# filrg/attackFL

Hardware: AMD Instinct MI355X
Metric: FL rounds/sec (whole node) + test-acc, TransformerModel/ICU, 8 clients (higher is better)
Workload: dtype bf16; 1 GPU; model=TransformerModel, global_batch=1024, seq_len=1, parallelism=fl8-clients-over-1-ranks, clients=8, local_epochs=5, rows_per_client=12000-15000, mode=fedavg, trainer=fused

## Files before the change

### attackfl_amd/fl/trainers.py

```python
from __future__ import annotations

from dataclasses import dataclass
from typing import List, Optional, Sequence, Tuple

import time

import torch

from ..data import DeviceTable
from ..models import ParamLayout, build_model
from ..utils.log import print_with_color


@dataclass
class Plan:

    order: torch.Tensor
    nd: torch.Tensor
    epochs: int
    nd_dev: Optional[torch.Tensor] = None

    def client(self, c: int) -> torch.Tensor:
        return self.order[c, :, : int(self.nd[c])]

# ... 288 lines not shown

        def fin():
            while not done.query():
                time.sleep(0)
            okh = buf[:, 0].to(torch.int32)
            if bool((okh < 0).any()):
                raise RuntimeError(f"{what}: a cross-workgroup hand-off timed out (workgroups not co-resident?)")
            return [bool(x) for x in okh.tolist()], buf[:, 1:].clone()

        return Pending(fin, ok, losses)

    def _readback(self, ok: torch.Tensor, losses: torch.Tensor):
        dev = self.device
        main = torch.cuda.current_stream(dev)
        cus = torch.cuda.get_device_properties(dev).multi_processor_count
        side = 3 * ok.shape[0] * 2 <= cus
        if side:
            rs = _RB_STREAMS.get(dev)
            if rs is None:
                rs = _RB_STREAMS[dev] = torch.cuda.Stream(device=dev)
            trained = torch.cuda.Event()
            trained.record(main)
            rs.wait_event(trained)
            ok.record_stream(rs)
            losses.record_stream(rs)
        else:
            rs = main
        return self._ring.read_back(ok, losses, rs)


class OracleTrainer:
# ... 104 lines not shown
```

### attackfl_amd/ops/transformer.py

```python
from __future__ import annotations

import os
from typing import Dict, List, Sequence, Tuple

import numpy as np
import torch
import torch.nn.functional as F

from . import native
from .rnn import _dev_i32, _on

NPARAM = 47693
M32 = 0xFFFFFFFF


def auto_split(C: int, dev) -> int:
    from ..parallel.launcher import gpu_sharers

    cus = torch.cuda.get_device_properties(dev).multi_processor_count // gpu_sharers()
    return 4 if cus >= 3 else 1


def client_chunks(C: int, cap: int) -> List[Tuple[int, int]]:
    if C <= 0:
        return []
    n = -(-C // max(1, cap))
    size = -(-C // n)
    return [(a, min(C, a + size)) for a in range(0, C, size)]


def onchip_capacity(dev, wgs_per_client: int = 3) -> int:
    from ..parallel.launcher import gpu_sharers

    cus = torch.cuda.get_device_properties(dev).multi_processor_count // gpu_sharers()
    cap = max(1, cus // wgs_per_client)
# ... 23 lines not shown
    dev = params.device
    C = params.shape[0]
    if split is None:
        split = int(os.environ.get("AFL_TF_SPLIT", "0") or 0) or (auto_split(C, dev) if C > 0 else 1)
    nd_t = _dev_i32(nd, dev)
    seeds_t = seeds if _on(seeds, dev) else torch.tensor([device_seed(s) for s in seeds], dtype=torch.int32, device=dev)
    kt = None
    if split == 4:
        kt = adam_step_table(float(lr), int(epochs) * -(-int(order.shape[2]) // int(batch)), dev)
    rows_c, order_c = rows.contiguous(), order.contiguous()

    def launch(p, o, n, s, first=True):
        return native().tf_train(p, rows_c, o, n, s, int(epochs), int(batch), float(lr), int(opt_mode),
                                 stamps if first else None, int(split), kt)
    if split == 4:
        return chunked(launch, C, onchip_capacity(dev, 3), params, order_c, nd_t, seeds_t)
    return launch(params, order_c, nd_t, seeds_t)


_KT_CACHE: Dict[tuple, torch.Tensor] = {}


def adam_step_table(lr: float, steps: int, dev) -> torch.Tensor:
    key = (lr, str(dev))
    t = _KT_CACHE.get(key)
    if t is None or t.shape[0] < steps:
        n = 1 << max(10, (max(steps, 1) - 1).bit_length())
        tt = np.arange(1, n + 1, dtype=np.float64)
        tab = np.stack([lr / (1.0 - 0.9 ** tt), 1.0 / np.sqrt(1.0 - 0.999 ** tt)], axis=1).astype(np.float32)
        t = _KT_CACHE[key] = torch.from_numpy(tab).to(dev)
    return t
# ... 160 lines not shown
```

### csrc/bindings.cpp

```cpp
#include <torch/extension.h>
#include <ATen/hip/HIPContext.h>

#include "kernels.h"

void afl_register_layers(pybind11::module& m);
void afl_register_ipc(pybind11::module& m);
void afl_register_har(pybind11::module& m);

namespace {

hipStream_t cur() { return at::hip::getCurrentHIPStream().stream(); }

bool sync_check() {
  static const bool on = [] {
    const char* e = getenv("AFL_SYNC_CHECK");
    return e && e[0] == '1';
  }();
  return on;
}
#define AFL_CHECK_LAUNCH()                                                              \
  do {                                                                                 \
    hipError_t e_ = hipGetLastError();                                                 \
    TORCH_CHECK(e_ == hipSuccess, "HIP launch failed: ", hipGetErrorString(e_));       \
    if (sync_check()) {                                                                \
// ... 683 lines not shown
  check_dev(order, "order", torch::kInt32);
  check_dev(nd, "nd", torch::kInt32);
  check_dev(seeds, "seeds", torch::kInt32);
  const long P = kind == 0 ? afl_tf_param_count() : afl_rnn_param_count();
  TORCH_CHECK(params.dim() == 2 && params.size(1) == P, "params must be [C, ", P, "]");
  TORCH_CHECK(rows.dim() == 2 && rows.size(1) == 24, "rows must be [N, 24]");
  const int C = params.size(0);
  TORCH_CHECK(order.dim() == 3 && order.size(0) == C && order.size(1) == epochs, "order must be [C, E, maxnd]");
  TORCH_CHECK(batch >= 2 && batch <= 128, "fused trainer supports batch sizes 2..128");
  TORCH_CHECK(kind == 1 || (split >= 1 && split <= 4), "TransformerModel trainer split must be 1..4, got ", split);
  const bool tf2 = kind == 0 && split == 4, rnn2 = kind == 1 && split == 4;
  const long wsf = tf2 ? afl_tf2_ws_floats() : rnn2 ? afl_rnn2_ws_floats() : kind == 0 ? afl_tf_ws_floats() : afl_rnn_ws_floats();
  const long stride = ((wsf + 63) / 64) * 64;
  auto ws = torch::empty({(long)C * stride}, params.options());
  const int split_eff = kind == 1 ? 3 : (int)std::max<int64_t>(1, split);
  const long sync_words = split_eff > 1 ? (long)C * (tf2 || rnn2 ? AFL_TF2_SYNC_WORDS : AFL_TF_SYNC_WORDS) : 0;
  const long head = ((long)C + (long)C * epochs + 3) / 4 * 4;
  auto zero = torch::zeros({head + sync_words}, order.options());
  auto ok = zero.narrow(0, 0, C);
  auto losses = zero.narrow(0, C, (long)C * epochs).view(torch::kFloat32).view({(long)C, epochs});
  if (C == 0) return {ok, losses};
  AflTfTrainArgs a;
  a.params = params.data_ptr<float>();
  a.rows = rows.data_ptr<float>();
  a.order = order.data_ptr<int>();
  a.nd = nd.data_ptr<int>();
  a.seeds = (const uint32_t*)seeds.data_ptr<int>();
  a.ws = ws.data_ptr<float>();
  a.ws_stride = stride;
  a.ok = ok.data_ptr<int>();
  a.losses = losses.data_ptr<float>();
// ... 11 lines not shown
  }
  a.sync = nullptr;
  a.kt = nullptr;
  a.kt_n = 0;
  if (kt.has_value() && kt->defined()) {
    check_dev(*kt, "kt", torch::kFloat32);
    TORCH_CHECK(kt->dim() == 2 && kt->size(1) == 2, "kt must be [steps, 2]");
    a.kt = kt->data_ptr<float>();
    a.kt_n = (int)kt->size(0);
  }
  a.split = split_eff;
  a.cpad = 0;
  if (a.split > 1) a.sync = (uint32_t*)zero.data_ptr<int>() + head;
  const int rc = tf2 ? afl_tf2_train(&a, cur()) : rnn2 ? afl_rnn2_train(&a, cur())
                 : kind == 0 ? afl_tf_train(&a, cur()) : afl_rnn_train(&a, cur());
  TORCH_CHECK(rc != -4, "branch-parallel fused trainer needs split * C <= CUs (all workgroups resident at once): "
              "launch at most onchip_capacity() clients at a time (ops/transformer.py chunked; AFL_MAX_CLIENTS_PER_LAUNCH "
              "caps it)");
  TORCH_CHECK(rc != -5, "on-chip trainer: Adam step table (kt) missing or shorter than the round");
  TORCH_CHECK(rc == 0, "fused trainer launch failed (", rc, ")");
  AFL_CHECK_LAUNCH();
  return {ok, losses};
}

std::vector<torch::Tensor> tf_train(torch::Tensor params, torch::Tensor rows, torch::Tensor order, torch::Tensor nd,
                                    torch::Tensor seeds, int64_t epochs, int64_t batch, double lr,
                                    int64_t opt_mode, c10::optional<torch::Tensor> stamps, int64_t split,
                                    c10::optional<torch::Tensor> kt) {
  return fused_train(0, params, rows, order, nd, seeds, epochs, batch, lr, opt_mode, stamps, split, kt);
}

std::vector<torch::Tensor> rnn_train(torch::Tensor params, torch::Tensor rows, torch::Tensor order, torch::Tensor nd,
                                     torch::Tensor seeds, int64_t epochs, int64_t batch, double lr, int64_t opt_mode,
// ... 94 lines not shown
  m.def("spec_eval", &spec_eval);
  m.def("spec_bisect", &spec_bisect);
  m.def("bisect_vec", &bisect_vec);
  m.def("weighted_rows", &weighted_rows, pybind11::arg("U"), pybind11::arg("w"), pybind11::arg("ok") = pybind11::none(),
        pybind11::arg("fallback") = pybind11::none());
  m.def("coord_select", &coord_select);
  m.def("row_dots", &row_dots);
  m.def("gmm_filter", &gmm_filter, pybind11::arg("G"), pybind11::arg("att"), pybind11::arg("rank") = 0);
  m.def("top_pc", &top_pc);
  m.def("krum_select", &krum_select);
  m.def("agr_bisect", &agr_bisect);
  m.def("dnc_run", &dnc_run);
  m.def("bulyan_coord", &bulyan_coord);
  m.def("geomed_weights", &geomed_weights);
  m.def("fxsum_test", &fxsum_test);
  m.def("gram_centred", &gram_centred);
  m.def("stoch_quant", &stoch_quant);
  m.def("adam_flat", &adam_flat);
  m.def("roc_auc", &roc_auc);
  m.def("roc_auc_dev", &roc_auc_dev);
  m.def("tf_eval_many", &tf_eval_many);
  m.def("hyper_delta_vjp", &hyper_delta_vjp);
  m.def("hyper_generate", &hyper_generate);
  m.def("hyper_adam_outer", &hyper_adam_outer);
  m.def("hyper_server_update", &hyper_server_update);
  m.def("make_plan", &make_plan);
  m.def("step_tables", &step_tables);
  m.def("hyper_features", &hyper_features);
  m.def("hyper_generate_many", &hyper_generate_many);
  m.def("hyper_small_capacity", &afl_hyper_small_capacity);
// ... 16 lines not shown
```

### csrc/kernels.h

```cpp
#pragma once
#include <hip/hip_runtime.h>
#include <stdint.h>

void afl_colstats(const float* G, int K, long P, float* mean, float* stdv, float* out, float z, int mode,
                  hipStream_t s);
void afl_weighted_rows(const float* U, const double* w, int N, long P, float* out, hipStream_t s,
                       const int* ok = nullptr, const float* fallback = nullptr);
int afl_pair_sqdist_nblocks(long P);
int afl_pair_sqdist(const float* G, int K, long P, double* partial, double* D, hipStream_t s);
void afl_seg_reduce(int mode, const float* X, long P, int rows, const float* mean, const float* dev, const int* tiles,
                    int T, const int* segf, int S, double* partial, double* out0, double* out1, hipStream_t s);
void afl_coord_select(const float* U, int N, long P, int mode, int trim, float* out, hipStream_t s);
int afl_row_dots_nchunks(long P);
void afl_row_dots(const float* U, const float* ref, int N, long P, int mode, double* partial, double* out,
                  hipStream_t s);
long afl_stoch_quant_ws(int N);
void afl_stoch_quant(const float* U, int N, long P, uint64_t seed, float* sigma, float* smin, float* smax,
                     float* ws, hipStream_t s);
void afl_adam_flat(float* p, const float* g, float* m, float* v, long n, int step, float lr, float b1, float b2,
                   float eps, float gscale, hipStream_t s);

int afl_hyper_nblocks(long P);
void afl_hyper_rows(const float* W, const float* b, const float* f, const float* u, long P, int H, float* out,
                    float* partial, float* dfeat, hipStream_t s);
// ... 63 lines not shown
  uint64_t* stamps;
  uint32_t* sync;
  int split;
  const float* kt;
  int kt_n;
  int cpad;
};
int afl_tf_train(const AflTfTrainArgs* a, hipStream_t s);
int afl_tf_eval_bf(const float* params, unsigned short* bf, const float* rows, int n, float* out, hipStream_t s);
int afl_tf_eval_many(const float* params, long pstride, unsigned short* bf, long bfstride, int C, const float* rows,
                     int n, float* out, hipStream_t s);
long afl_tf_ws_floats();
constexpr int AFL_TF_SYNC_WORDS = 4 * 8 * 32 + 32;
constexpr int AFL_GR_WORDS = 2 * 2 * 8 * 1024;
constexpr int AFL_TF2_SYNC_WORDS = AFL_TF_SYNC_WORDS + AFL_GR_WORDS;
int afl_tf2_train(const AflTfTrainArgs* a, hipStream_t s);
int afl_tf2_train_stamped(const AflTfTrainArgs* a, hipStream_t s);
long afl_tf2_ws_floats();
int afl_fxsum_test(const float* vals, int W, uint32_t seed, int mode, float* out, hipStream_t s);
int afl_rnn_train(const AflTfTrainArgs* a, hipStream_t s);
long afl_rnn_ws_floats();
int afl_rnn2_train(const AflTfTrainArgs* a, hipStream_t s);
int afl_rnn2_train_stamped(const AflTfTrainArgs* a, hipStream_t s);
long afl_rnn2_ws_floats();
int afl_rnn2_eval(const float* params, long pstride, int C, const float* rows, int n, float* out, hipStream_t s);
int afl_rnn_param_count();
int afl_tf_bf_ushorts();
int afl_tf_param_count();

struct AflDrop {
  const uint32_t* seeds;
// ... 301 lines not shown
```

### csrc/kernels/tf2.hip

```cpp
#include "common.h"
#include "kernels.h"
#include "tf_common.h"
#include "fused_common.h"
#define ONCHIP_NO_AGPR
#include "onchip.h"

using namespace tf;

namespace t2 {

using namespace oc;



constexpr int LDDN = 24 * 2, LDVO = LD64 + 16;
constexpr int B_IMG_D = 0;
constexpr int B_IMG_V = B_IMG_D + 64 * LDDN;
constexpr int B_IMG_O = B_IMG_V + 64 * LDVO;
constexpr int B_IMG_F1 = B_IMG_O + 64 * LDVO;
constexpr int B_IMG_F2 = B_IMG_F1 + 16 * LD64;
constexpr int B_H0 = B_IMG_F2 + 64 * LD32;
constexpr int B_A = B_H0 + 16384;
constexpr int B_X1N = B_A + 16384;
constexpr int B_DF3 = B_X1N + 16384;
// ... 21 lines not shown
#endif
#ifndef TF2_HLD2
#define TF2_HLD2 (LD64 + 16)
#endif
constexpr int HLD1 = TF2_HLD1, HLD2 = TF2_HLD2;
constexpr int H_IMG_W1 = 0;
constexpr int H_IMG_W2 = H_IMG_W1 + 64 * HLD1;
constexpr int H_CAT = H_IMG_W2 + 32 * HLD2;
constexpr int H_A1 = H_CAT + 32768;
constexpr int H_DZ1 = H_A1 + 16384;
constexpr int H_DZ2 = H_DZ1 + 16384;
constexpr int H_NVEC = 132;
constexpr int H_VEC = H_DZ2 + 8192;
constexpr int H_PART = H_VEC + H_NVEC * 4;
constexpr int H_LOSS = H_PART + 8 * H_NVEC * 4;
constexpr int H_TOTAL = H_LOSS + 64;
enum { HV_B1 = 0, HV_B2 = 64, HV_WO = 96, HV_BO = 128 };

constexpr int SMEM_CORE = B_TOTAL > H_TOTAL ? B_TOTAL : H_TOTAL;
#ifdef TF2_STAMPS
constexpr int ST_OFF = SMEM_CORE, ST_N = 16;
constexpr int SMEM = ST_OFF + ST_N * 8;
#else
constexpr int SMEM = SMEM_CORE;
#endif
static_assert(SMEM <= 160 * 1024, "LDS budget");

constexpr int MOM_SLOTS = 11;
constexpr long WS_MOM = 0;
constexpr long MOM_WG_BYTES = (long)MOM_SLOTS * NTH * 16;
constexpr int CMP_SLOTS = 1;
constexpr long BR_UNITS = (long)CMP_SLOTS * NTH * 16;
constexpr long BR_SMALL = BR_UNITS + 8L * 12 * 64 * 16;
constexpr long BR_WG_BYTES = BR_SMALL + 4L * 9 * 64 * 16;
constexpr long WS_BYTES = WS_MOM + MOM_WG_BYTES + 2 * BR_WG_BYTES;

__device__ __forceinline__ void ln_colsum(uchar* smem, int k, const float (&x)[16], int lane) {
  float s;
  const int f = colsum64(x, lane, s);
  lds_addq(smem + B_DBL, 64 * k + f, s);
}
__host__ __device__ constexpr int ln_seg(int k) { return k < 2 ? VS_G1 + k : VS_G2 + (k - 2); }
static_assert(ln_seg(0) == VS_G1 && ln_seg(1) == VS_B1 && ln_seg(2) == VS_G2 && ln_seg(3) == VS_B2 &&
              ln_seg(4) == VS_G3 && ln_seg(5) == VS_B3, "DBL order");

__device__ __forceinline__ uint32_t mask16(uint32_t key, uint32_t layer, int r, int g, uint32_t thr) {
  uint32_t m = 0;
#pragma unroll
  for (int t = 0; t < 4; ++t) {
#pragma unroll
// ... 787 lines not shown
  (void)stp; (void)a; (void)smem;
}
__device__ __forceinline__ void stamp_fini(Stamp& stp, const AflTfTrainArgs& a, uchar* smem, int tid) {
#ifdef TF2_STAMPS
  if (stp.on && tid == 0)
    for (int i = 0; i < ST_N - 1; ++i) a.stamps[i] = *(LDS_AS uint64_t*)(smem + ST_OFF + 8 * i);
#endif
  (void)stp; (void)a; (void)smem; (void)tid;
}

template <int BR>
__device__ __forceinline__ void branch_main(const AflTfTrainArgs& a, int cid, uchar* smem) {
  const int tid = threadIdx.x, lane = tid & 63, wave = __builtin_amdgcn_readfirstlane(tid >> 6), g = lane >> 4;
  float* P = a.params + (long)cid * NPARAM;
  uchar* ws = (uchar*)(a.ws + (long)cid * a.ws_stride);
  gu32* sync = (gu32*)(a.sync + (long)cid * AFL_TF2_SYNC_WORDS);
  const __amdgpu_buffer_rsrc_t rg = gr_rsrc(sync);
  for (int i = tid; i < SMEM / 4; i += NTH) ldsf(smem, 0)[i] = 0.f;
  __syncthreads();
  BrState st;
  const __amdgpu_buffer_rsrc_t rm = rsrc(ws + WS_MOM + MOM_WG_BYTES + BR * BR_WG_BYTES);
  br_init<BR>(smem, st, P, rm, lane, wave, tid);
  asm volatile("s_waitcnt vmcnt(0)" ::: "memory");
  __syncthreads();
  Stamp stp;
  stamp_init(stp, a, smem);

  const int nd = a.nd[cid], BS = a.batch, E = a.E;
  const uint32_t seed = a.seeds[cid];
  LDS_AS uint32_t* abort_w = ldsu(smem, B_MISC);
  int step = 0;
// ... 81 lines not shown
  stamp_fini(stp, a, smem, tid);
  br_fini<BR>(st, P, rm, lane, wave, tid);
}

constexpr Mat HW1{FC1_W, 64, 128, H_IMG_W1, HLD1};
constexpr Mat HW2{FC2_W, 32, 64, H_IMG_W2, HLD2};
__device__ __forceinline__ int hvec_param(int e) {
  return e < 64 ? FC1_B + e : e < 96 ? FC2_B + (e - 64) : e < 128 ? OUT_W + (e - 96) : e == 128 ? OUT_B : -1;
}
struct HdState {
  TS blk[4];
  TS t2;
  VS vec;
};

__device__ __forceinline__ void head_main(const AflTfTrainArgs& a, int cid, uchar* smem) {
  const int tid = threadIdx.x, lane = tid & 63, wave = __builtin_amdgcn_readfirstlane(tid >> 6), g = lane >> 4;
  const int r = 16 * wave + (lane & 15);
  float* P = a.params + (long)cid * NPARAM;
  uchar* ws = (uchar*)(a.ws + (long)cid * a.ws_stride);
  gu32* sync = (gu32*)(a.sync + (long)cid * AFL_TF2_SYNC_WORDS);
  const __amdgpu_buffer_rsrc_t rg = gr_rsrc(sync);
  for (int i = tid; i < SMEM / 4; i += NTH) ldsf(smem, 0)[i] = 0.f;
  __syncthreads();
  HdState st;
  Stamp stp;
  const __amdgpu_buffer_rsrc_t rm = rsrc(ws + WS_MOM);
  mom_zero(rm, tid);
  {
    const int Ta = 2 * (wave & 3), Tb = 2 * (wave >> 2);
#pragma unroll
    for (int x = 0; x < 2; ++x)
#pragma unroll
      for (int y = 0; y < 2; ++y) tile_load(st.blk[2 * x + y], HW1, Ta + x, Tb + y, lane, P, smem);
    tile_load(st.t2, HW2, wave & 3, wave >> 2, lane, P, smem);
    float p0 = 0.f;
    if (tid < H_NVEC) {
      const int pi = hvec_param(tid);
      p0 = pi >= 0 ? P[pi] : 0.f;
      ldsf(smem, H_VEC)[tid] = p0;
    }
    st.vec = VS{aw(p0)};
  }
  __syncthreads();
  stamp_init(stp, a, smem);

  const int nd = a.nd[cid], BS = a.batch, E = a.E;
  const int nb_total = (nd + BS - 1) / BS;
  const uint32_t seed = a.seeds[cid];
  const uchar* vec = smem + H_VEC;
  LDS_AS float* part = ldsf(smem, H_PART) + wave * H_NVEC;
  LDS_AS float* lossw = ldsf(smem, H_LOSS);
  int step = 0;
  bool failed = false, timed_out = false;
  float epoch_loss = 0.f;
  Walk w{0, 0};
  int cur_e = 0;
  bool more = walk_valid(w, nd, BS, E);
  float lab = 0.f;
  auto load_lab = [&](const Walk& ww) {
    const int Bn = min(BS, nd - ww.b0);
    const gi32* ord = (const gi32*)(a.order + ((long)cid * E + ww.e) * a.maxnd);
    lab = r < Bn ? ((const gf*)a.rows)[(long)ord[ww.b0 + r] * ROW + ROW - 1] : 0.f;
  };
  if (more) load_lab(w);
  while (more) {
    while (cur_e < w.e) {
      if (tid == 0) a.losses[(long)cid * E + cur_e] = epoch_loss / (float)max(nb_total, 1);
      epoch_loss = 0.f;
      ++cur_e;
    }
    ++step;
    const AdamK K = adam_k(a, step);
    const uint32_t key = afl_hash32(seed, (uint32_t)step);
    const int Bn = min(BS, nd - w.b0);
    const bool valid = r < Bn;
    const float inv_bn = 1.f / (float)Bn;
    const uint32_t mh = mask16(key, L_HEAD, r, g, THR_P03);
    sb();
    u32x4 cv[4];
    const int go[2] = {gr_off(0, 0, wave, lane), gr_off(0, 1, wave, lane)};
    const uint32_t fv = gr_get<2>(rg, go, cv, (uint32_t)step, 0, sync + XF_TMO, lane);
    if (fv == 0xFFFFFFFFu) {
      timed_out = failed = true;
      break;
    }
    prio_hi();
    stp(10, tid);
    float a1[16], gk1[16];
    {
      f4v acc[4];
#pragma unroll
      for (int T = 0; T < 4; ++T) {
        acc[T] = Z4;
#pragma unroll
        for (int s = 0; s < 4; ++s)
          acc[T] = mma(wfrag(smem + H_IMG_W1, HLD1, T, s, lane), __builtin_bit_cast(s8v, cv[s]), acc[T]);
      }
      float b1[16];
      vec16(b1, vec + HV_B1 * 4, g);
#pragma unroll
      for (int t = 0; t < 4; ++t)
#pragma unroll
        for (int i = 0; i < 4; i += 2) {
          const int j = 4 * t + i;
          gf2v gp;
          const gf2v gl = gelu2(gf2v{acc[t][i] + b1[j], acc[t][i + 1] + b1[j + 1]}, gp);
#pragma unroll
          for (int h = 0; h < 2; ++h) {
            a1[j + h] = keepf(gl[h] * INV_K03, mh, j + h);
            gk1[j + h] = keepf(gp[h] * INV_K03, mh, j + h);
          }
        }
    }
    float dz2[8], gw[8];
    float dy3 = 0.f, pl = 0.f;
    {
      const s8v b0 = bfrag(a1, 0), b1 = bfrag(a1, 1);
      f4v acc[2];
#pragma unroll
      for (int T = 0; T < 2; ++T) {
        acc[T] = mma(wfrag(smem + H_IMG_W2, HLD2, T, 0, lane), b0, Z4);
        acc[T] = mma(wfrag(smem + H_IMG_W2, HLD2, T, 1, lane), b1, acc[T]);
      }
      float b2[8], wo[8], g2[8], gp2[8];
      vec8(b2, vec + HV_B2 * 4, g);
      vec8(wo, vec + HV_WO * 4, g);
      float dot = 0.f;
#pragma unroll
      for (int t = 0; t < 2; ++t)
#pragma unroll
        for (int i = 0; i < 4; i += 2) {
          const int j = 4 * t + i;
          gf2v gp;
          const gf2v gl = gelu2(gf2v{acc[t][i] + b2[j], acc[t][i + 1] + b2[j + 1]}, gp);
          g2[j] = gl[0];
          g2[j + 1] = gl[1];
          gp2[j] = gp[0];
          gp2[j + 1] = gp[1];
          dot += g2[j] * wo[j];
          dot += g2[j + 1] * wo[j + 1];
        }
      const float y3 = fk::rsum4(dot) + *(const LDS_AS float*)(vec + HV_BO * 4);
      const float p = sigmoidf_(y3);
      if (valid) {
        const float pq = p * (1.f - p);
        dy3 = (p - lab) * (pq >= 1e-12f ? 1.f : pq * 1e12f) * inv_bn;
      }
      pl = p;
#pragma unroll
      for (int j = 0; j < 8; ++j) {
        dz2[j] = dy3 * wo[j] * gp2[j];
        gw[j] = dy3 * g2[j];
      }
    }
    const uint32_t wave_nan = __builtin_amdgcn_ballot_w64(!(fabsf(dy3) <= 3.402823466e38f)) != 0 ? 1u : 0u;
    float dz1[16];
    {
      const s8v bz = bfrag(dz2, 0);
#pragma unroll
      for (int T = 0; T < 4; ++T) {
        const f4v acc = mma(wtfrag<true>(smem + H_IMG_W2, HLD2, T, 0, lane), bz, Z4);
#pragma unroll
        for (int i = 0; i < 4; ++i) dz1[4 * T + i] = acc[i] * gk1[4 * T + i];
      }
    }
    {
      const s8v b0 = bfrag(dz1, 0), b1 = bfrag(dz1, 1);
#pragma unroll
      for (int hb = 0; hb < 2; ++hb) {
        float d[16];
#pragma unroll
        for (int Tl = 0; Tl < 4; ++Tl) {
          const int T = 4 * hb + Tl;
          f4v acc = mma(wtfrag<true>(smem + H_IMG_W1, HLD1, T, 0, lane), b0, Z4);
          acc = mma(wtfrag<true>(smem + H_IMG_W1, HLD1, T, 1, lane), b1, acc);
#pragma unroll
          for (int i = 0; i < 4; ++i) d[4 * Tl + i] = acc[i];
        }
        u32x4 u[2];
        pack16(d, u);
        gr_put(rg, gr_off(1, hb, wave, lane), u, ((uint32_t)step << 1) | wave_nan);
      }
    }
    prio_lo();
    {
      float lrow = 0.f;
      if (valid) {
        float lg, lg1;
        bce_logs(pl, lg, lg1);
        const float lp = lg < -100.f ? -100.f : lg, l1p = lg1 < -100.f ? -100.f : lg1;
        lrow = -(lab * lp + (1.f - lab) * l1p);
      }
      const float lsum = wave_sum(g == 0 ? lrow : 0.f);
      if (lane == 0) {
        lossw[wave] = lsum;
        lossw[8 + wave] = __uint_as_float(wave_nan);
      }
    }
    {
      sb();
#pragma unroll
      for (int t = 0; t < 8; ++t) {
        const u32x4 u = cv[t >> 1];
        const u32x2v v = (t & 1) ? u32x2v{u[2], u[3]} : u32x2v{u[0], u[1]};
        *(LDS_AS u32x2v*)(smem + H_CAT + t128(r, 4 * t + g)) = v;
      }
#pragma unroll
      for (int t = 0; t < 4; ++t) st4<TK64>(smem + H_A1, r, 4 * t + g, a1 + 4 * t);
#pragma unroll
      for (int t = 0; t < 2; ++t) st4<TK32>(smem + H_DZ2, r, 4 * t + g, dz2 + 4 * t);
#pragma unroll
      for (int t = 0; t < 4; ++t) st4<TK64>(smem + H_DZ1, r, 4 * t + g, dz1 + 4 * t);
      float sb2, swo, sb1;
      const int f2 = colsum32(dz2, lane, sb2), fo = colsum32(gw, lane, swo);
      if (f2 >= 0) {
        part[HV_B2 + f2] = sb2;
        part[HV_WO + fo] = swo;
      }
      const int f1 = colsum64(dz1, lane, sb1);
      part[HV_B1 + f1] = sb1;
      const float dbo = wave_sum(g == 0 ? dy3 : 0.f);
      if (lane == 0) part[HV_BO] = dbo;
    }
    stp(11, tid);
    f4v hm[6], hv[6];
#pragma unroll
    for (int k = 0; k < 4; ++k) {
      hm[k] = mom_ld(rm, k, tid);
      hv[k] = mom_ld(rm, 4 + k, tid);
    }
    hm[4] = mom_ld(rm, 8, tid);
    hv[4] = mom_ld(rm, 9, tid);
    hm[5] = mom_ld(rm, 10, tid);
    Walk wn = w;
    wn.b0 += BS;
    more = walk_valid(wn, nd, BS, E);
    lds_bar();
// ... 57 lines not shown
      for (int k = 0; k < 4; ++k) {
        mom_st(rm, k, tid, hm[k]);
        mom_st(rm, 4 + k, tid, hv[k]);
      }
      mom_st(rm, 8, tid, hm[4]);
      mom_st(rm, 9, tid, hv[4]);
      mom_st(rm, 10, tid, hm[5]);
    }
    stp(13, tid);
    lds_bar();
    stp(14, tid);
  }
  stamp_fini(stp, a, smem, tid);
  if (!failed) {
    while (cur_e < E) {
      if (tid == 0) a.losses[(long)cid * E + cur_e] = epoch_loss / (float)max(nb_total, 1);
      epoch_loss = 0.f;
      ++cur_e;
    }
  }
  {
    int ln = lane, wv = wave;
    opq(ln, wv);
    const int Ta = 2 * (wv & 3), Tb = 2 * (wv >> 2);
#pragma unroll
    for (int x = 0; x < 2; ++x)
#pragma unroll
      for (int y = 0; y < 2; ++y) tile_store(st.blk[2 * x + y], HW1, Ta + x, Tb + y, ln, P);
    tile_store(st.t2, HW2, wv & 3, wv >> 2, ln, P);
    if (tid < H_NVEC && hvec_param(tid) >= 0) P[hvec_param(tid)] = ar(st.vec.p);
  }
  if (tid == 0) {
    const bool tmo = timed_out || __hip_atomic_load(sync + XF_TMO, __ATOMIC_RELAXED, __HIP_MEMORY_SCOPE_AGENT);
    a.ok[cid] = tmo ? -1 : (failed ? 0 : 1);
  }
}

}

#ifdef TF2_STAMPS
#define K_TF2 k_tf2_train_stamped
#else
#define K_TF2 k_tf2_train
#endif
__global__ void __launch_bounds__(t2::NTH) K_TF2(AflTfTrainArgs a) {
  extern __shared__ __attribute__((aligned(16))) unsigned char smem[];
  const int cp = a.cpad > 0 ? a.cpad : a.C;
  const int role = blockIdx.x / cp, cid = blockIdx.x - role * cp;
  if (cid >= a.C) return;
#if defined(TF2_ROLE)
  if (TF2_ROLE == 0) t2::head_main(a, cid, smem);
  else if (TF2_ROLE == 1) t2::branch_main<0>(a, cid, smem);
  else t2::branch_main<1>(a, cid, smem);
  (void)role;
#else
  if (role == 0)
    t2::head_main(a, cid, smem);
  else if (role == 1)
    t2::branch_main<0>(a, cid, smem);
  else
    t2::branch_main<1>(a, cid, smem);
#endif
}

#ifndef TF2_STAMPS
__global__ void __launch_bounds__(1024) k_fxsum_test(const float* __restrict__ vals, int W, uint32_t seed, int mode,
                                                   float* __restrict__ out) {
  __shared__ double q[64];
  const int lane = threadIdx.x & 63, w = threadIdx.x >> 6;
  if (threadIdx.x < 64) q[threadIdx.x] = 0;
  __syncthreads();
  const uint32_t spins = afl_hash32(seed, (uint32_t)w) & 1023u;
  for (uint32_t i = 0; i < spins; ++i) __builtin_amdgcn_s_sleep(1);
// ... 6 lines not shown
  if (threadIdx.x < 64)
    out[lane] = mode == 0 ? oc::lds_getq((const oc::uchar*)q, lane)
                          : (float)((LDS_AS double*)q)[lane];
}
int afl_fxsum_test(const float* vals, int W, uint32_t seed, int mode, float* out, hipStream_t s) {
  if (W < 1 || W > 8) return -1;
  hipLaunchKernelGGL(k_fxsum_test, dim3(1), dim3(64 * W), 0, s, vals, W, seed, mode, out);
  return (int)hipGetLastError();
}
#endif

#ifdef TF2_STAMPS
int afl_tf2_train_stamped(const AflTfTrainArgs* a, hipStream_t s) {
#else
long afl_tf2_ws_floats() { return t2::WS_BYTES / 4; }

int afl_tf2_train(const AflTfTrainArgs* a, hipStream_t s) {
  if (a->stamps) return afl_tf2_train_stamped(a, s);
#endif
  if (a->batch > 128 || a->batch < 2 || !a->sync) return -1;
  if (!a->kt || a->kt_n < a->E * ((a->maxnd + a->batch - 1) / a->batch)) return -5;
  if (hipFuncSetAttribute((const void*)K_TF2, hipFuncAttributeMaxDynamicSharedMemorySize, t2::SMEM) != hipSuccess) return -2;
  int dev = 0, cus = 0;
  if (hipGetDevice(&dev) != hipSuccess || hipDeviceGetAttribute(&cus, hipDeviceAttributeMultiprocessorCount, dev) != hipSuccess)
    return -3;
  const int wgs = 3;
  if (wgs * a->C > cus) return -4;
  AflTfTrainArgs b = *a;
  b.cpad = (a->C + 7) / 8 * 8;
#ifdef TF2_NO_PAD
  b.cpad = a->C;
#endif
  if (wgs * b.cpad > cus) b.cpad = a->C;
  hipLaunchKernelGGL(K_TF2, dim3(wgs * b.cpad), dim3(t2::NTH), t2::SMEM, s, b);
  return 0;
}
```

Baseline: 127.7 rounds/s.

## Split TransformerModel head workgroup into two halves sharing activations via export slots

The head role of the on-chip TransformerModel trainer now runs on two workgroups per client instead of one, giving four workgroups per client. In each, waves 0-3 compute the forward/backward pass for four row tiles. They export their activations, gradients and partial sums through new global exchange slots so the other half's remaining waves can rebuild the LDS state without recomputing. Each half keeps its own Adam moment buffer, and the Python launch sizing and readback-stream decision now query the per-client workgroup count. The intent is to halve the serial critical-path work in the head, at the cost of more CUs per client, extra cross-workgroup hand-off traffic, and fewer clients fitting per launch.

```diff
diff --git a/attackfl_amd/fl/trainers.py b/attackfl_amd/fl/trainers.py
--- a/attackfl_amd/fl/trainers.py
+++ b/attackfl_amd/fl/trainers.py
@@ -326,7 +326,8 @@
         dev = self.device
         main = torch.cuda.current_stream(dev)
         cus = torch.cuda.get_device_properties(dev).multi_processor_count
-        side = 3 * ok.shape[0] * 2 <= cus
+        wgs = 3 if self.model_name == "RNNModel" else self.T.tf2_wgs()
+        side = wgs * ok.shape[0] * 2 <= cus
         if side:
             rs = _RB_STREAMS.get(dev)
             if rs is None:
diff --git a/attackfl_amd/ops/transformer.py b/attackfl_amd/ops/transformer.py
--- a/attackfl_amd/ops/transformer.py
+++ b/attackfl_amd/ops/transformer.py
@@ -14,11 +14,16 @@
 M32 = 0xFFFFFFFF
 
 
+def tf2_wgs() -> int:
+    f = getattr(native(), "tf2_wgs_per_client", None)
+    return int(f()) if f is not None else 3
+
+
 def auto_split(C: int, dev) -> int:
     from ..parallel.launcher import gpu_sharers
 
     cus = torch.cuda.get_device_properties(dev).multi_processor_count // gpu_sharers()
-    return 4 if cus >= 3 else 1
+    return 4 if cus >= tf2_wgs() else 1
 
 
 def client_chunks(C: int, cap: int) -> List[Tuple[int, int]]:
@@ -72,7 +77,7 @@
         return native().tf_train(p, rows_c, o, n, s, int(epochs), int(batch), float(lr), int(opt_mode),
                                  stamps if first else None, int(split), kt)
     if split == 4:
-        return chunked(launch, C, onchip_capacity(dev, 3), params, order_c, nd_t, seeds_t)
+        return chunked(launch, C, onchip_capacity(dev, tf2_wgs()), params, order_c, nd_t, seeds_t)
     return launch(params, order_c, nd_t, seeds_t)
 
 
diff --git a/csrc/bindings.cpp b/csrc/bindings.cpp
--- a/csrc/bindings.cpp
+++ b/csrc/bindings.cpp
@@ -721,7 +721,8 @@
   const long stride = ((wsf + 63) / 64) * 64;
   auto ws = torch::empty({(long)C * stride}, params.options());
   const int split_eff = kind == 1 ? 3 : (int)std::max<int64_t>(1, split);
-  const long sync_words = split_eff > 1 ? (long)C * (tf2 || rnn2 ? AFL_TF2_SYNC_WORDS : AFL_TF_SYNC_WORDS) : 0;
+  const long sync_words =
+      split_eff > 1 ? (long)C * (tf2 ? AFL_TF2H_SYNC_WORDS : rnn2 ? AFL_TF2_SYNC_WORDS : AFL_TF_SYNC_WORDS) : 0;
   const long head = ((long)C + (long)C * epochs + 3) / 4 * 4;
   auto zero = torch::zeros({head + sync_words}, order.options());
   auto ok = zero.narrow(0, 0, C);
@@ -763,9 +764,10 @@
   if (a.split > 1) a.sync = (uint32_t*)zero.data_ptr<int>() + head;
   const int rc = tf2 ? afl_tf2_train(&a, cur()) : rnn2 ? afl_rnn2_train(&a, cur())
                  : kind == 0 ? afl_tf_train(&a, cur()) : afl_rnn_train(&a, cur());
-  TORCH_CHECK(rc != -4, "branch-parallel fused trainer needs split * C <= CUs (all workgroups resident at once): "
-              "launch at most onchip_capacity() clients at a time (ops/transformer.py chunked; AFL_MAX_CLIENTS_PER_LAUNCH "
-              "caps it)");
+  TORCH_CHECK(rc != -4, "branch-parallel fused trainer needs workgroups-per-client * C <= CUs (all workgroups resident at "
+              "once; tf2: tf2_wgs_per_client() = ", afl_tf2_wgs_per_client(), ", otherwise the split): launch at most "
+              "onchip_capacity(dev, workgroups per client) clients at a time (ops/transformer.py chunked; "
+              "AFL_MAX_CLIENTS_PER_LAUNCH caps it)");
   TORCH_CHECK(rc != -5, "on-chip trainer: Adam step table (kt) missing or shorter than the round");
   TORCH_CHECK(rc == 0, "fused trainer launch failed (", rc, ")");
   AFL_CHECK_LAUNCH();
@@ -890,6 +892,7 @@
   m.def("bulyan_coord", &bulyan_coord);
   m.def("geomed_weights", &geomed_weights);
   m.def("fxsum_test", &fxsum_test);
+  m.def("tf2_wgs_per_client", &afl_tf2_wgs_per_client);
   m.def("gram_centred", &gram_centred);
   m.def("stoch_quant", &stoch_quant);
   m.def("adam_flat", &adam_flat);
diff --git a/csrc/kernels.h b/csrc/kernels.h
--- a/csrc/kernels.h
+++ b/csrc/kernels.h
@@ -101,7 +101,10 @@
 constexpr int AFL_TF_SYNC_WORDS = 4 * 8 * 32 + 32;
 constexpr int AFL_GR_WORDS = 2 * 2 * 8 * 1024;
 constexpr int AFL_TF2_SYNC_WORDS = AFL_TF_SYNC_WORDS + AFL_GR_WORDS;
+constexpr int AFL_EX_WORDS = 2 * 8 * 5 * 1024;
+constexpr int AFL_TF2H_SYNC_WORDS = AFL_TF2_SYNC_WORDS + AFL_EX_WORDS;
 int afl_tf2_train(const AflTfTrainArgs* a, hipStream_t s);
+int afl_tf2_wgs_per_client();
 int afl_tf2_train_stamped(const AflTfTrainArgs* a, hipStream_t s);
 long afl_tf2_ws_floats();
 int afl_fxsum_test(const float* vals, int W, uint32_t seed, int mode, float* out, hipStream_t s);
diff --git a/csrc/kernels/tf2.hip b/csrc/kernels/tf2.hip
--- a/csrc/kernels/tf2.hip
+++ b/csrc/kernels/tf2.hip
@@ -59,7 +59,8 @@
 constexpr int H_VEC = H_DZ2 + 8192;
 constexpr int H_PART = H_VEC + H_NVEC * 4;
 constexpr int H_LOSS = H_PART + 8 * H_NVEC * 4;
-constexpr int H_TOTAL = H_LOSS + 64;
+constexpr int H_CNT = H_LOSS + 64;
+constexpr int H_TOTAL = H_CNT + 16;
 enum { HV_B1 = 0, HV_B2 = 64, HV_WO = 96, HV_BO = 128 };
 
 constexpr int SMEM_CORE = B_TOTAL > H_TOTAL ? B_TOTAL : H_TOTAL;
@@ -78,7 +79,8 @@
 constexpr long BR_UNITS = (long)CMP_SLOTS * NTH * 16;
 constexpr long BR_SMALL = BR_UNITS + 8L * 12 * 64 * 16;
 constexpr long BR_WG_BYTES = BR_SMALL + 4L * 9 * 64 * 16;
-constexpr long WS_BYTES = WS_MOM + MOM_WG_BYTES + 2 * BR_WG_BYTES;
+constexpr long WS_MOM2 = WS_MOM + MOM_WG_BYTES + 2 * BR_WG_BYTES;
+constexpr long WS_BYTES = WS_MOM2 + MOM_WG_BYTES;
 
 __device__ __forceinline__ void ln_colsum(uchar* smem, int k, const float (&x)[16], int lane) {
   float s;
@@ -896,7 +898,7 @@
   const int tid = threadIdx.x, lane = tid & 63, wave = __builtin_amdgcn_readfirstlane(tid >> 6), g = lane >> 4;
   float* P = a.params + (long)cid * NPARAM;
   uchar* ws = (uchar*)(a.ws + (long)cid * a.ws_stride);
-  gu32* sync = (gu32*)(a.sync + (long)cid * AFL_TF2_SYNC_WORDS);
+  gu32* sync = (gu32*)(a.sync + (long)cid * AFL_TF2H_SYNC_WORDS);
   const __amdgpu_buffer_rsrc_t rg = gr_rsrc(sync);
   for (int i = tid; i < SMEM / 4; i += NTH) ldsf(smem, 0)[i] = 0.f;
   __syncthreads();
@@ -1008,18 +1010,28 @@
   VS vec;
 };
 
-__device__ __forceinline__ void head_main(const AflTfTrainArgs& a, int cid, uchar* smem) {
+constexpr int NWG = 4;
+constexpr int EX_SLOTS = 5;
+constexpr int EX_BASE = 2 * GR_DIR_BYTES;
+static_assert(EX_BASE == AFL_GR_WORDS * 4 && 2 * 8 * EX_SLOTS * 1024 == AFL_EX_WORDS, "export slots follow the hand-off slots");
+__device__ __forceinline__ int ex_off(int parity, int tile, int k, int lane) {
+  return EX_BASE + ((parity * 8 + tile) * EX_SLOTS + k) * 4096 + lane * 16;
+}
+
+__device__ __forceinline__ void head_main(const AflTfTrainArgs& a, int cid, uchar* smem, int half) {
   const int tid = threadIdx.x, lane = tid & 63, wave = __builtin_amdgcn_readfirstlane(tid >> 6), g = lane >> 4;
-  const int r = 16 * wave + (lane & 15);
+  const bool crit = wave < 4;
+  const int tile = crit ? 4 * half + wave : 4 * (1 - half) + (wave - 4);
+  const int r = 16 * tile + (lane & 15);
   float* P = a.params + (long)cid * NPARAM;
   uchar* ws = (uchar*)(a.ws + (long)cid * a.ws_stride);
-  gu32* sync = (gu32*)(a.sync + (long)cid * AFL_TF2_SYNC_WORDS);
+  gu32* sync = (gu32*)(a.sync + (long)cid * AFL_TF2H_SYNC_WORDS);
   const __amdgpu_buffer_rsrc_t rg = gr_rsrc(sync);
   for (int i = tid; i < SMEM / 4; i += NTH) ldsf(smem, 0)[i] = 0.f;
   __syncthreads();
   HdState st;
   Stamp stp;
-  const __amdgpu_buffer_rsrc_t rm = rsrc(ws + WS_MOM);
+  const __amdgpu_buffer_rsrc_t rm = rsrc(ws + (half == 0 ? WS_MOM : WS_MOM2));
   mom_zero(rm, tid);
   {
     const int Ta = 2 * (wave & 3), Tb = 2 * (wave >> 2);
@@ -1043,7 +1055,6 @@
   const int nb_total = (nd + BS - 1) / BS;
   const uint32_t seed = a.seeds[cid];
   const uchar* vec = smem + H_VEC;
-  LDS_AS float* part = ldsf(smem, H_PART) + wave * H_NVEC;
   LDS_AS float* lossw = ldsf(smem, H_LOSS);
   int step = 0;
   bool failed = false, timed_out = false;
@@ -1060,140 +1071,223 @@
   if (more) load_lab(w);
   while (more) {
     while (cur_e < w.e) {
-      if (tid == 0) a.losses[(long)cid * E + cur_e] = epoch_loss / (float)max(nb_total, 1);
+      if (tid == 0 && half == 0) a.losses[(long)cid * E + cur_e] = epoch_loss / (float)max(nb_total, 1);
       epoch_loss = 0.f;
       ++cur_e;
     }
     ++step;
     const AdamK K = adam_k(a, step);
-    const uint32_t key = afl_hash32(seed, (uint32_t)step);
     const int Bn = min(BS, nd - w.b0);
-    const bool valid = r < Bn;
-    const float inv_bn = 1.f / (float)Bn;
-    const uint32_t mh = mask16(key, L_HEAD, r, g, THR_P03);
-    sb();
     u32x4 cv[4];
-    const int go[2] = {gr_off(0, 0, wave, lane), gr_off(0, 1, wave, lane)};
-    const uint32_t fv = gr_get<2>(rg, go, cv, (uint32_t)step, 0, sync + XF_TMO, lane);
-    if (fv == 0xFFFFFFFFu) {
-      timed_out = failed = true;
-      break;
-    }
-    prio_hi();
-    stp(10, tid);
-    float a1[16], gk1[16];
-    {
-      f4v acc[4];
-#pragma unroll
-      for (int T = 0; T < 4; ++T) {
-        acc[T] = Z4;
-#pragma unroll
-        for (int s = 0; s < 4; ++s)
-          acc[T] = mma(wfrag(smem + H_IMG_W1, HLD1, T, s, lane), __builtin_bit_cast(s8v, cv[s]), acc[T]);
-      }
-      float b1[16];
-      vec16(b1, vec + HV_B1 * 4, g);
-#pragma unroll
-      for (int t = 0; t < 4; ++t)
-#pragma unroll
-        for (int i = 0; i < 4; i += 2) {
-          const int j = 4 * t + i;
-          gf2v gp;
-          const gf2v gl = gelu2(gf2v{acc[t][i] + b1[j], acc[t][i + 1] + b1[j + 1]}, gp);
-#pragma unroll
-          for (int h = 0; h < 2; ++h) {
-            a1[j + h] = keepf(gl[h] * INV_K03, mh, j + h);
-            gk1[j + h] = keepf(gp[h] * INV_K03, mh, j + h);
+    u32x4 a1w[2], dz1w[2], dz2w;
+    float lsum = 0.f;
+    uint32_t wave_nan = 0u;
+    const int par = step & 1;
+    if (crit) {
+      const uint32_t key = afl_hash32(seed, (uint32_t)step);
+      const bool valid = r < Bn;
+      const float inv_bn = 1.f / (float)Bn;
+      const uint32_t mh = mask16(key, L_HEAD, r, g, THR_P03);
+      sb();
+      const int go[2] = {gr_off(0, 0, tile, lane), gr_off(0, 1, tile, lane)};
+      const uint32_t fv = gr_get<2>(rg, go, cv, (uint32_t)step, 0, sync + XF_TMO, lane);
+      if (fv == 0xFFFFFFFFu) {
+        lds_signal(smem, H_CNT, lane);
+        timed_out = failed = true;
+        break;
+      }
+      prio_hi();
+      stp(10, tid);
+      float a1[16], gk1[16];
+      {
+        f4v acc[4];
+#pragma unroll
+        for (int T = 0; T < 4; ++T) {
+          acc[T] = Z4;
+#pragma unroll
+          for (int s = 0; s < 4; ++s)
+            acc[T] = mma(wfrag(smem + H_IMG_W1, HLD1, T, s, lane), __builtin_bit_cast(s8v, cv[s]), acc[T]);
+        }
+        float b1[16];
+        vec16(b1, vec + HV_B1 * 4, g);
+#pragma unroll
+        for (int t = 0; t < 4; ++t)
+#pragma unroll
+          for (int i = 0; i < 4; i += 2) {
+            const int j = 4 * t + i;
+            gf2v gp;
+            const gf2v gl = gelu2(gf2v{acc[t][i] + b1[j], acc[t][i + 1] + b1[j + 1]}, gp);
+#pragma unroll
+            for (int h = 0; h < 2; ++h) {
+              a1[j + h] = keepf(gl[h] * INV_K03, mh, j + h);
+              gk1[j + h] = keepf(gp[h] * INV_K03, mh, j + h);
+            }
           }
+      }
+      float dz2[8], gw[8];
+      float dy3 = 0.f, pl = 0.f;
+      {
+        const s8v b0 = bfrag(a1, 0), b1 = bfrag(a1, 1);
+        f4v acc[2];
+#pragma unroll
+        for (int T = 0; T < 2; ++T) {
+          acc[T] = mma(wfrag(smem + H_IMG_W2, HLD2, T, 0, lane), b0, Z4);
+          acc[T] = mma(wfrag(smem + H_IMG_W2, HLD2, T, 1, lane), b1, acc[T]);
         }
-    }
-    float dz2[8], gw[8];
-    float dy3 = 0.f, pl = 0.f;
-    {
-      const s8v b0 = bfrag(a1, 0), b1 = bfrag(a1, 1);
-      f4v acc[2];
-#pragma unroll
-      for (int T = 0; T < 2; ++T) {
-        acc[T] = mma(wfrag(smem + H_IMG_W2, HLD2, T, 0, lane), b0, Z4);
-        acc[T] = mma(wfrag(smem + H_IMG_W2, HLD2, T, 1, lane), b1, acc[T]);
-      }
-      float b2[8], wo[8], g2[8], gp2[8];
-      vec8(b2, vec + HV_B2 * 4, g);
-      vec8(wo, vec + HV_WO * 4, g);
-      float dot = 0.f;
-#pragma unroll
-      for (int t = 0; t < 2; ++t)
-#pragma unroll
-        for (int i = 0; i < 4; i += 2) {
-          const int j = 4 * t + i;
-          gf2v gp;
-          const gf2v gl = gelu2(gf2v{acc[t][i] + b2[j], acc[t][i + 1] + b2[j + 1]}, gp);
-          g2[j] = gl[0];
-          g2[j + 1] = gl[1];
-          gp2[j] = gp[0];
-          gp2[j + 1] = gp[1];
-          dot += g2[j] * wo[j];
-          dot += g2[j + 1] * wo[j + 1];
+        float b2[8], wo[8], g2[8], gp2[8];
+        vec8(b2, vec + HV_B2 * 4, g);
+        vec8(wo, vec + HV_WO * 4, g);
+        float dot = 0.f;
+#pragma unroll
+        for (int t = 0; t < 2; ++t)
+#pragma unroll
+          for (int i = 0; i < 4; i += 2) {
+            const int j = 4 * t + i;
+            gf2v gp;
+            const gf2v gl = gelu2(gf2v{acc[t][i] + b2[j], acc[t][i + 1] + b2[j + 1]}, gp);
+            g2[j] = gl[0];
+            g2[j + 1] = gl[1];
+            gp2[j] = gp[0];
+            gp2[j + 1] = gp[1];
+            dot += g2[j] * wo[j];
+            dot += g2[j + 1] * wo[j + 1];
+          }
+        const float y3 = fk::rsum4(dot) + *(const LDS_AS float*)(vec + HV_BO * 4);
+        const float p = sigmoidf_(y3);
+        if (valid) {
+          const float pq = p * (1.f - p);
+          dy3 = (p - lab) * (pq >= 1e-12f ? 1.f : pq * 1e12f) * inv_bn;
         }
-      const float y3 = fk::rsum4(dot) + *(const LDS_AS float*)(vec + HV_BO * 4);
-      const float p = sigmoidf_(y3);
-      if (valid) {
-        const float pq = p * (1.f - p);
-        dy3 = (p - lab) * (pq >= 1e-12f ? 1.f : pq * 1e12f) * inv_bn;
-      }
-      pl = p;
-#pragma unroll
-      for (int j = 0; j < 8; ++j) {
-        dz2[j] = dy3 * wo[j] * gp2[j];
-        gw[j] = dy3 * g2[j];
-      }
-    }
-    const uint32_t wave_nan = __builtin_amdgcn_ballot_w64(!(fabsf(dy3) <= 3.402823466e38f)) != 0 ? 1u : 0u;
-    float dz1[16];
-    {
-      const s8v bz = bfrag(dz2, 0);
-#pragma unroll
-      for (int T = 0; T < 4; ++T) {
-        const f4v acc = mma(wtfrag<true>(smem + H_IMG_W2, HLD2, T, 0, lane), bz, Z4);
-#pragma unroll
-        for (int i = 0; i < 4; ++i) dz1[4 * T + i] = acc[i] * gk1[4 * T + i];
-      }
-    }
-    {
-      const s8v b0 = bfrag(dz1, 0), b1 = bfrag(dz1, 1);
-#pragma unroll
-      for (int hb = 0; hb < 2; ++hb) {
-        float d[16];
-#pragma unroll
-        for (int Tl = 0; Tl < 4; ++Tl) {
-          const int T = 4 * hb + Tl;
-          f4v acc = mma(wtfrag<true>(smem + H_IMG_W1, HLD1, T, 0, lane), b0, Z4);
-          acc = mma(wtfrag<true>(smem + H_IMG_W1, HLD1, T, 1, lane), b1, acc);
-#pragma unroll
-          for (int i = 0; i < 4; ++i) d[4 * Tl + i] = acc[i];
+        pl = p;
+#pragma unroll
+        for (int j = 0; j < 8; ++j) {
+          dz2[j] = dy3 * wo[j] * gp2[j];
+          gw[j] = dy3 * g2[j];
         }
-        u32x4 u[2];
-        pack16(d, u);
-        gr_put(rg, gr_off(1, hb, wave, lane), u, ((uint32_t)step << 1) | wave_nan);
-      }
-    }
-    prio_lo();
-    {
-      float lrow = 0.f;
-      if (valid) {
-        float lg, lg1;
-        bce_logs(pl, lg, lg1);
-        const float lp = lg < -100.f ? -100.f : lg, l1p = lg1 < -100.f ? -100.f : lg1;
-        lrow = -(lab * lp + (1.f - lab) * l1p);
-      }
-      const float lsum = wave_sum(g == 0 ? lrow : 0.f);
-      if (lane == 0) {
-        lossw[wave] = lsum;
-        lossw[8 + wave] = __uint_as_float(wave_nan);
-      }
+      }
+      wave_nan = __builtin_amdgcn_ballot_w64(!(fabsf(dy3) <= 3.402823466e38f)) != 0 ? 1u : 0u;
+      float dz1[16];
+      {
+        const s8v bz = bfrag(dz2, 0);
+#pragma unroll
+        for (int T = 0; T < 4; ++T) {
+          const f4v acc = mma(wtfrag<true>(smem + H_IMG_W2, HLD2, T, 0, lane), bz, Z4);
+#pragma unroll
+          for (int i = 0; i < 4; ++i) dz1[4 * T + i] = acc[i] * gk1[4 * T + i];
+        }
+      }
+      {
+        const s8v b0 = bfrag(dz1, 0), b1 = bfrag(dz1, 1);
+#pragma unroll
+        for (int hb = 0; hb < 2; ++hb) {
+          float d[16];
+#pragma unroll
+          for (int Tl = 0; Tl < 4; ++Tl) {
+            const int T = 4 * hb + Tl;
+            f4v acc = mma(wtfrag<true>(smem + H_IMG_W1, HLD1, T, 0, lane), b0, Z4);
+            acc = mma(wtfrag<true>(smem + H_IMG_W1, HLD1, T, 1, lane), b1, acc);
+#pragma unroll
+            for (int i = 0; i < 4; ++i) d[4 * Tl + i] = acc[i];
+          }
+          u32x4 u[2];
+          pack16(d, u);
+          gr_put(rg, gr_off(1, hb, tile, lane), u, ((uint32_t)step << 1) | wave_nan);
+        }
+      }
+      prio_lo();
+      lds_signal(smem, H_CNT, lane);
+      pack16(a1, a1w);
+      pack16(dz1, dz1w);
+      dz2w = u32x4{pk2(dz2[0], dz2[1]), pk2(dz2[2], dz2[3]), pk2(dz2[4], dz2[5]), pk2(dz2[6], dz2[7])};
+      const uint32_t xtag = ((uint32_t)step << 1) | wave_nan;
+      int xl = lane, xt = tile;
+      asm volatile("" : "+v"(xl));
+      asm volatile("" : "+s"(xt));
+      const int xo = ex_off(par, xt, 0, xl);
+      {
+        const u32x4 c0[2] = {cv[0], cv[1]}, c1[2] = {cv[2], cv[3]};
+        gr_put(rg, xo, c0, xtag);
+        gr_put(rg, xo + 4096, c1, xtag);
+        gr_put(rg, xo + 2 * 4096, a1w, xtag);
+        gr_put(rg, xo + 3 * 4096, dz1w, xtag);
+      }
+      {
+        float lrow = 0.f;
+        if (valid) {
+          float lg, lg1;
+          bce_logs(pl, lg, lg1);
+          const float lp = lg < -100.f ? -100.f : lg, l1p = lg1 < -100.f ? -100.f : lg1;
+          lrow = -(lab * lp + (1.f - lab) * l1p);
+        }
+        lsum = wave_sum(xl < 16 ? lrow : 0.f);
+      }
+      {
+        sb();
+        LDS_AS float* pt = ldsf(smem, H_PART) + xt * H_NVEC;
+        float sb2, swo, sb1;
+        const int f2 = colsum32(dz2, xl, sb2), fo = colsum32(gw, xl, swo);
+        if (f2 >= 0) {
+          pt[HV_B2 + f2] = sb2;
+          pt[HV_WO + fo] = swo;
+        }
+        const int f1 = colsum64(dz1, xl, sb1);
+        pt[HV_B1 + f1] = sb1;
+        const float dbo = wave_sum(xl < 16 ? dy3 : 0.f);
+        if (xl == 0) pt[HV_BO] = dbo;
+        const LDS_AS float* pr = pt + xl;
+        const float p0 = pr[0], p1 = pr[64], p2 = xl < 4 ? pr[128] : 0.f;
+        const u32x4 c4[2] = {dz2w, u32x4{__float_as_uint(p0), __float_as_uint(p1), __float_as_uint(p2), __float_as_uint(lsum)}};
+        gr_put(rg, xo + 4 * 4096, c4, xtag);
+      }
+    } else {
+      prio_lo();
+      if (!lds_wait(smem, H_CNT, 4u * (uint32_t)step)) {
+        if (lane == 0) __hip_atomic_store(sync + XF_TMO, 1u, __ATOMIC_RELAXED, __HIP_MEMORY_SCOPE_AGENT);
+        timed_out = failed = true;
+        break;
+      }
+      stp(10, tid);
+      int xl = lane, xt = tile;
+      asm volatile("" : "+v"(xl));
+      asm volatile("" : "+s"(xt));
+      const int xo = ex_off(par, xt, 0, xl);
+      const int eb[2] = {xo + 3 * 4096, xo + 4 * 4096};
+      u32x4 eu[4];
+      const uint32_t fv = gr_get<2>(rg, eb, eu, (uint32_t)step, 1, sync + XF_TMO, lane);
+      if (fv == 0xFFFFFFFFu) {
+        timed_out = failed = true;
+        break;
+      }
+      dz1w[0] = eu[0];
+      dz1w[1] = eu[1];
+      dz2w = eu[2];
+      LDS_AS float* pw = ldsf(smem, H_PART) + xt * H_NVEC + xl;
+      pw[0] = __uint_as_float(eu[3][0]);
+      pw[64] = __uint_as_float(eu[3][1]);
+      if (xl < 4) pw[128] = __uint_as_float(eu[3][2]);
+      lsum = __uint_as_float(eu[3][3]);
+      wave_nan = fv & 1u;
+      const int ea[3] = {xo, xo + 4096, xo + 2 * 4096};
+      u32x4 ev[6];
+      if (gr_get<3>(rg, ea, ev, (uint32_t)step, 1, sync + XF_TMO, lane) == 0xFFFFFFFFu) {
+        timed_out = failed = true;
+        break;
+      }
+#pragma unroll
+      for (int k = 0; k < 4; ++k) cv[k] = ev[k];
+      a1w[0] = ev[4];
+      a1w[1] = ev[5];
     }
     {
       sb();
+      int sl = lane, stl = tile;
+      asm volatile("" : "+v"(sl));
+      asm volatile("" : "+s"(stl));
+      const int r = 16 * stl + (sl & 15), g = sl >> 4;
+      if (sl == 0) {
+        lossw[stl] = lsum;
+        lossw[8 + stl] = __uint_as_float(wave_nan);
+      }
 #pragma unroll
       for (int t = 0; t < 8; ++t) {
         const u32x4 u = cv[t >> 1];
@@ -1201,21 +1295,13 @@
         *(LDS_AS u32x2v*)(smem + H_CAT + t128(r, 4 * t + g)) = v;
       }
 #pragma unroll
-      for (int t = 0; t < 4; ++t) st4<TK64>(smem + H_A1, r, 4 * t + g, a1 + 4 * t);
-#pragma unroll
-      for (int t = 0; t < 2; ++t) st4<TK32>(smem + H_DZ2, r, 4 * t + g, dz2 + 4 * t);
-#pragma unroll
-      for (int t = 0; t < 4; ++t) st4<TK64>(smem + H_DZ1, r, 4 * t + g, dz1 + 4 * t);
-      float sb2, swo, sb1;
-      const int f2 = colsum32(dz2, lane, sb2), fo = colsum32(gw, lane, swo);
-      if (f2 >= 0) {
-        part[HV_B2 + f2] = sb2;
-        part[HV_WO + fo] = swo;
-      }
-      const int f1 = colsum64(dz1, lane, sb1);
-      part[HV_B1 + f1] = sb1;
-      const float dbo = wave_sum(g == 0 ? dy3 : 0.f);
-      if (lane == 0) part[HV_BO] = dbo;
+      for (int t = 0; t < 4; ++t) {
+        const int q = 2 * (t & 1);
+        *(LDS_AS u32x2v*)(smem + H_A1 + t64(r, 4 * t + g)) = u32x2v{a1w[t >> 1][q], a1w[t >> 1][q + 1]};
+        *(LDS_AS u32x2v*)(smem + H_DZ1 + t64(r, 4 * t + g)) = u32x2v{dz1w[t >> 1][q], dz1w[t >> 1][q + 1]};
+      }
+#pragma unroll
+      for (int t = 0; t < 2; ++t) *(LDS_AS u32x2v*)(smem + H_DZ2 + t32(r, 4 * t + g)) = u32x2v{dz2w[2 * t], dz2w[2 * t + 1]};
     }
     stp(11, tid);
     f4v hm[6], hv[6];
@@ -1303,11 +1389,12 @@
   stamp_fini(stp, a, smem, tid);
   if (!failed) {
     while (cur_e < E) {
-      if (tid == 0) a.losses[(long)cid * E + cur_e] = epoch_loss / (float)max(nb_total, 1);
+      if (tid == 0 && half == 0) a.losses[(long)cid * E + cur_e] = epoch_loss / (float)max(nb_total, 1);
       epoch_loss = 0.f;
       ++cur_e;
     }
   }
+  if (half != 0) return;
   {
     int ln = lane, wv = wave;
     opq(ln, wv);
@@ -1338,14 +1425,14 @@
   const int role = blockIdx.x / cp, cid = blockIdx.x - role * cp;
   if (cid >= a.C) return;
 #if defined(TF2_ROLE)
-  if (TF2_ROLE == 0) t2::head_main(a, cid, smem);
-  else if (TF2_ROLE == 1) t2::branch_main<0>(a, cid, smem);
+  if (TF2_ROLE < 2) t2::head_main(a, cid, smem, TF2_ROLE);
+  else if (TF2_ROLE == 2) t2::branch_main<0>(a, cid, smem);
   else t2::branch_main<1>(a, cid, smem);
   (void)role;
 #else
-  if (role == 0)
-    t2::head_main(a, cid, smem);
-  else if (role == 1)
+  if (role < 2)
+    t2::head_main(a, cid, smem, role);
+  else if (role == 2)
     t2::branch_main<0>(a, cid, smem);
   else
     t2::branch_main<1>(a, cid, smem);
@@ -1382,6 +1469,7 @@
 int afl_tf2_train_stamped(const AflTfTrainArgs* a, hipStream_t s) {
 #else
 long afl_tf2_ws_floats() { return t2::WS_BYTES / 4; }
+int afl_tf2_wgs_per_client() { return t2::NWG; }
 
 int afl_tf2_train(const AflTfTrainArgs* a, hipStream_t s) {
   if (a->stamps) return afl_tf2_train_stamped(a, s);
@@ -1392,7 +1480,7 @@
   int dev = 0, cus = 0;
   if (hipGetDevice(&dev) != hipSuccess || hipDeviceGetAttribute(&cus, hipDeviceAttributeMultiprocessorCount, dev) != hipSuccess)
     return -3;
-  const int wgs = 3;
+  const int wgs = t2::NWG;
   if (wgs * a->C > cus) return -4;
   AflTfTrainArgs b = *a;
   b.cpad = (a->C + 7) / 8 * 8;
```

After: 129.7 rounds/s, median of 6. 1.02x the previous value.
